# scottjones03/NoisyQuantumSimulator

Measured on AMD Instinct MI355X. Metric: Lindblad param-points/sec (2-atom Rydberg CZ sweep); achieved HBM GB/s vs peak, higher is better.
Workload: dtype f64; 1 GPU; C2: 10k-point (Omega, Delta) LP-square CZ sweep per GPU, medium apparatus, full reference noise model (8 Lindblad channels); points_per_gpu=10000, global_points=10000, parallelism=range-shard x1, method=chebyshev (auto: 16-lane DPP-row propagator kernel, phase frame)

## Files before the change

### noisyquantumsimulator_amd/csrc/ryd_engine.hip

```cpp
#include <hip/hip_runtime.h>

#include <dlfcn.h>

#include <math.h>
#include <stdint.h>
#include <stdio.h>
#include <string.h>

#include <algorithm>
#include <atomic>
#include <chrono>
#include <complex>
#include <condition_variable>
#include <mutex>
#include <string>
#include <thread>
#include <utility>
#include <vector>

#include "../../include/ryd_engine.h"

struct ryd_slot_work {
  void* dbuf = nullptr;
  size_t dcap = 0;
// ... 100 lines not shown
    g.om_re = pulse ? a * q.xr : a;
    g.om_im = pulse ? a * q.xi : 0.0;
    g.dl = q.Dl;
    g.dt = q.tau / (double)n_steps;
  } else if (PROTO == RYD_PROTO_SMOOTH_JP) {
    const double dt = q.tau / (double)n_steps;
    const double tm = (double)s * dt + dt / 2;
    const double ph = q.A * cos(q.wmod * tm - q.phoff);
    double sn, cs;
    sincos(ph, &sn, &cs);
    g.om_re = q.Om * cs;
    g.om_im = q.Om * sn;
    g.dl = q.Dl;
    g.dt = dt;
  } else {
    if (s >= q.nseg) {
      g.om_re = g.om_im = g.dl = g.dt = 0.0;
      return g;
    }
    const double b0 = s == 0 ? 0.0 : col(q.prm, RYD_P_SWT0 + s - 1, q.ld, q.i) / q.Om;
    const double b1 = (s + 1 == q.nseg) ? q.otau / q.Om : col(q.prm, RYD_P_SWT0 + s, q.ld, q.i) / q.Om;
    const double ph = col(q.prm, RYD_P_PHI0 + s, q.ld, q.i);
    double sn, cs;
    sincos(ph, &sn, &cs);
    g.om_re = q.Om * cs;
    g.om_im = q.Om * sn;
    g.dl = 0.0;
    double dt = b1 - b0;
    g.dt = dt < 1e-18 ? 0.0 : dt;
  }
  return g;
}

__device__ __forceinline__ void h_bounds(const Seg& g, double V, double d1, double& emin, double& emax) {
  const double e[3] = {0.0, d1, -g.dl};
  const double w = 0.5 * sqrt(g.om_re * g.om_re + g.om_im * g.om_im);
  emin = 1e300;
  emax = -1e300;
#pragma unroll
  for (int a1 = 0; a1 < 3; ++a1)
#pragma unroll
    for (int a2 = a1; a2 < 3; ++a2) {
      const double E = e[a1] + e[a2] + ((a1 == 2 && a2 == 2) ? V : 0.0);
      const double r = w * ((a1 ? 1.0 : 0.0) + (a2 ? 1.0 : 0.0));
      emin = fmin(emin, E - r);
      emax = fmax(emax, E + r);
    }
}

__device__ __forceinline__ int cheb_terms(double x) {
  if (x < 24.0) {
    double t = 1.0;
    int k = 0;
    do {
      ++k;
      t *= 0.5 * x / (double)k;
    } while (!(t < 1e-18 && (double)k > x));
    return k;
  }
  return (int)ceil(x + 12.0 * cbrt(x) + 10.0);
}

__device__ __forceinline__ int wave_max(int v) {
  v = max(v, __builtin_amdgcn_update_dpp(v, v, 0xB1, 0xF, 0xF, false));
  v = max(v, __builtin_amdgcn_update_dpp(v, v, 0x4E, 0xF, 0xF, false));
  v = max(v, __builtin_amdgcn_update_dpp(v, v, 0x141, 0xF, 0xF, false));
  v = max(v, __builtin_amdgcn_update_dpp(v, v, 0x140, 0xF, 0xF, false));
  const int a = __builtin_amdgcn_readlane(v, 0), b = __builtin_amdgcn_readlane(v, 16);
  const int c = __builtin_amdgcn_readlane(v, 32), d = __builtin_amdgcn_readlane(v, 48);
  return max(max(a, b), max(c, d));
}

struct Gen {
  double g0, g1, mg01, hx, hy, hx2, hy2, hz2, G;
};

__device__ __forceinline__ Gen make_gen(const Seg& g, double d1, const double* r, double s) {
  Gen a;
  const double hx = 0.5 * g.om_re, hy = -0.5 * g.om_im, hz = 0.5 * (d1 + g.dl);
  a.g0 = s * r[1];
// ... 1818 lines not shown
thread_local std::string g_err;

int fail(int code, const std::string& msg) {
  g_err = msg;
  return code;
}

#define HIPCHK(expr)                                                                       \
  do {                                                                                     \
    hipError_t _e = (expr);                                                                \
    if (_e != hipSuccess)                                                                  \
      return fail(RYD_ERR_HIP, std::string(#expr) + ": " + hipGetErrorString(_e));          \
  } while (0)

using KernelFn = void (*)(const double*, int64_t, int64_t, double*, int64_t, double*, int64_t,
                          uint32_t*, int, int);

bool use_propagator(const ryd_batch_desc* d) {
  const bool auto_prop = d->protocol == RYD_PROTO_LP_SQUARE || d->protocol == RYD_PROTO_BANGBANG ||
                         d->protocol == RYD_PROTO_SMOOTH_JP;
  return d->dim == 3 && d->evolution == RYD_EVOL_LINDBLAD &&
         (d->method == RYD_METHOD_CHEB_SQUARING || (d->method == RYD_METHOD_CHEBYSHEV && auto_prop));
}

bool use_sym16(const ryd_batch_desc* d) {
  const char* e = getenv("RYD_SYM16");
  if (e && e[0] == '0') return false;
  return d->dim == 3 && d->evolution == RYD_EVOL_LINDBLAD && d->method == RYD_METHOD_CHEBYSHEV &&
         (d->flags & RYD_FLAG_SYMMETRIC_ATOMS) != 0 &&
         (d->protocol == RYD_PROTO_LP_SQUARE || d->protocol == RYD_PROTO_BANGBANG ||
          d->protocol == RYD_PROTO_SMOOTH_JP);
}

bool use_shaped16(const ryd_batch_desc* d) {
  const char* e = getenv("RYD_SHAPED16");
  if (e && e[0] == '0') return false;
  return d->dim == 3 && d->evolution == RYD_EVOL_LINDBLAD && d->method == RYD_METHOD_CHEBYSHEV &&
         (d->flags & RYD_FLAG_SYMMETRIC_ATOMS) != 0 && d->protocol == RYD_PROTO_LP_SHAPED;
}

bool use_dim4_prop(const ryd_batch_desc* d) {
  const char* e = getenv("RYD_DIM4_PROP");
  if (e && e[0] == '0') return false;
  return d->dim == 4 && d->evolution == RYD_EVOL_LINDBLAD && d->method == RYD_METHOD_CHEBYSHEV &&
         (d->flags & RYD_FLAG_SYMMETRIC_ATOMS) != 0 &&
         (d->protocol == RYD_PROTO_LP_SQUARE || d->protocol == RYD_PROTO_BANGBANG ||
          d->protocol == RYD_PROTO_SMOOTH_JP);
}

bool use_ket_block(const ryd_batch_desc* d) {
  const char* e = getenv("RYD_KET_BLOCK");
  if (e && e[0] == '0') return false;
  return d->evolution == RYD_EVOL_KET && d->method == RYD_METHOD_CHEBYSHEV;
}

KernelFn pick_kernel(const ryd_batch_desc* d) {
  const bool sym = (d->flags & RYD_FLAG_SYMMETRIC_ATOMS) != 0;
  if (d->dim == 4) {
    if (d->evolution == RYD_EVOL_LINDBLAD) {
      switch (d->protocol) {
        case RYD_PROTO_LP_SQUARE:
          return sym ? lindblad4_cheb_kernel<RYD_PROTO_LP_SQUARE, true> : lindblad4_cheb_kernel<RYD_PROTO_LP_SQUARE, false>;
        case RYD_PROTO_LP_SHAPED:
          return sym ? lindblad4_cheb_kernel<RYD_PROTO_LP_SHAPED, true> : lindblad4_cheb_kernel<RYD_PROTO_LP_SHAPED, false>;
        case RYD_PROTO_BANGBANG:
          return sym ? lindblad4_cheb_kernel<RYD_PROTO_BANGBANG, true> : lindblad4_cheb_kernel<RYD_PROTO_BANGBANG, false>;
// ... 155 lines not shown
    int64_t ms = d->max_steps;
    void* args[] = {(void*)&dp, (void*)&n, (void*)&ldp, (void*)&ds, (void*)&lds, (void*)&dm,
                    (void*)&ldm, (void*)&dstat, (void*)&ns, (void*)&sh, (void*)&rt, (void*)&at,
                    (void*)&ms};
    HIPCHK(hipLaunchKernel((const void*)f, dim3((unsigned)blocks), dim3(DP_BLOCK), args, 0, stream));
    return RYD_OK;
  }
  if (use_dim4_prop(d)) {
    using PFn = void (*)(const double*, int64_t, int64_t, double*, int64_t, double*, int64_t, uint32_t*,
                         int, int);
    PFn f = d->protocol == RYD_PROTO_LP_SQUARE ? lindblad4_prop_kernel<RYD_PROTO_LP_SQUARE>
            : d->protocol == RYD_PROTO_SMOOTH_JP ? lindblad4_prop_kernel<RYD_PROTO_SMOOTH_JP>
                                                  : lindblad4_prop_kernel<RYD_PROTO_BANGBANG>;
    const int64_t blocks = (n + D4_PPB - 1) / D4_PPB;
    if (blocks > 0x7fffffffLL) return fail(RYD_ERR_INVALID, "batch too large for one launch");
    int ns = d->n_steps, sh = d->shape;
    void* args[] = {(void*)&dp, (void*)&n, (void*)&ldp, (void*)&ds, (void*)&lds, (void*)&dm,
                    (void*)&ldm, (void*)&dstat, (void*)&ns, (void*)&sh};
    HIPCHK(hipLaunchKernel((const void*)f, dim3((unsigned)blocks), dim3(D4_BLOCK), args, 0, stream));
    return RYD_OK;
  }
  if (use_shaped16(d)) {
    const int64_t blocks = (n + SH_PPW - 1) / SH_PPW;
    if (blocks > 0x7fffffffLL) return fail(RYD_ERR_INVALID, "batch too large for one launch");
    int ns = d->n_steps, sh = d->shape;
    void* args[] = {(void*)&dp, (void*)&n, (void*)&ldp, (void*)&ds, (void*)&lds, (void*)&dm,
                    (void*)&ldm, (void*)&dstat, (void*)&ns, (void*)&sh};
    HIPCHK(hipLaunchKernel((const void*)lindblad_shaped16_kernel<RYD_PROTO_LP_SHAPED>, dim3((unsigned)blocks),
                           dim3(SH_BLOCK), args, 0, stream));
    return RYD_OK;
  }
  if (use_sym16(d)) {
    using SFn = void (*)(const double*, int64_t, int64_t, double*, int64_t, double*, int64_t, uint32_t*,
                         int, int);
    SFn f = d->protocol == RYD_PROTO_LP_SQUARE ? lindblad_sym16_kernel<RYD_PROTO_LP_SQUARE>
            : d->protocol == RYD_PROTO_SMOOTH_JP ? lindblad_sym16_kernel<RYD_PROTO_SMOOTH_JP>
                                                  : lindblad_sym16_kernel<RYD_PROTO_BANGBANG>;
    const int64_t blocks = (n + S16_PPW - 1) / S16_PPW;
    if (blocks > 0x7fffffffLL) return fail(RYD_ERR_INVALID, "batch too large for one launch");
    int ns = d->n_steps, sh = d->shape;
    void* args[] = {(void*)&dp, (void*)&n, (void*)&ldp, (void*)&ds, (void*)&lds, (void*)&dm,
                    (void*)&ldm, (void*)&dstat, (void*)&ns, (void*)&sh};
    HIPCHK(hipLaunchKernel((const void*)f, dim3((unsigned)blocks), dim3(S16_BLOCK), args, 0, stream));
    return RYD_OK;
  }
  if (use_propagator(d) && d->protocol == RYD_PROTO_SMOOTH_JP && jp_split_enabled())
    return launch_jp_split(d, dp, n, ldp, ds, lds, dm, ldm, dstat, stream);
  KernelFn k = pick_kernel(d);
  if (!k) return fail(RYD_ERR_UNSUPPORTED, "no kernel for this descriptor");
  const int64_t blocks = use_propagator(d) ? (n + PPB - 1) / PPB
                        : use_ket_block(d) ? (n + BLOCK - 1) / BLOCK : (4 * n + BLOCK - 1) / BLOCK;
  if (blocks > 0x7fffffffLL) return fail(RYD_ERR_INVALID, "batch too large for one launch");
  int ns = d->n_steps, sh = d->shape;
  void* args[] = {(void*)&dp, (void*)&n, (void*)&ldp, (void*)&ds, (void*)&lds, (void*)&dm,
                  (void*)&ldm, (void*)&dstat, (void*)&ns, (void*)&sh};
  HIPCHK(hipLaunchKernel((const void*)k, dim3((unsigned)blocks), dim3(BLOCK), args, 0, stream));
  return RYD_OK;
}

bool coh_prop_enabled() {
  const char* e = getenv("RYD_COH_PROP");
  return !(e && e[0] == '0');
}

template <int PROTO>
int launch_coherences_proto(const double* dp, int64_t n, int64_t ldp, double* dc, int64_t ldc,
                            uint32_t* dstat, int ns, int sh, hipStream_t stream) {
  if (PROTO != RYD_PROTO_LP_SHAPED && coh_prop_enabled()) {
    const int64_t blocks = (n + CP_NR - 1) / CP_NR;
    if (blocks > 0x7fffffffLL) return fail(RYD_ERR_INVALID, "batch too large for one launch");
    void* args[] = {(void*)&dp, (void*)&n, (void*)&ldp, (void*)&dc, (void*)&ldc, (void*)&dstat, (void*)&ns, (void*)&sh};
    HIPCHK(hipLaunchKernel((const void*)coherence_prop_kernel<PROTO>, dim3((unsigned)blocks), dim3(CP_BLOCK), args, 0,
                           stream));
    return RYD_OK;
  }
// ... 751 lines not shown
```

### noisyquantumsimulator_amd/csrc/ryd_sym16.inc

```

constexpr int S16_BLOCK = 64;
constexpr int S16_PPW = 4;

#ifndef RYD_S16_SETPRIO
#define RYD_S16_SETPRIO 1
#endif
__device__ __forceinline__ bool s16_one_round() {
  return RYD_S16_SETPRIO && gridDim.x <= 256u * 4u * (unsigned)RYD_S16_WAVES;
}
#define S16_PRIO(n) do { if (s16_one_round()) __builtin_amdgcn_s_setprio(n); } while (0)
#ifndef RYD_S16_PRIO_SPLIT
#define RYD_S16_PRIO_SPLIT 1
#endif
#ifdef RYD_S16_PROF
#define S16_MARK(k) (s16_ts[k] = (double)__builtin_readcyclecounter())
#define S16_PROF_ARG , double* s16_ts
#define S16_PROF_PASS , s16_ts
#else
#define S16_MARK(k) ((void)0)
#define S16_PROF_ARG
#define S16_PROF_PASS
#endif

#ifndef RYD_XCD_MAP
#define RYD_XCD_MAP 2
#endif
__device__ __forceinline__ int64_t xcd_block(int64_t b, int64_t nb) {
  if (RYD_XCD_MAP == 0) return b;
  if (RYD_XCD_MAP == 1) {
    const int64_t q = nb / 8, rem = nb % 8, x = b % 8, k = b / 8;
    return x * q + (x < rem ? x : rem) + k;
  }
  const int64_t full = (nb / 32) * 32;
  if (b >= full) return b;
  const int64_t x = b % 8, k = b / 8;
  return ((k / 4) * 8 + x) * 4 + (k % 4);
}

template <int K>
__device__ __forceinline__ double row_bcast(double v) {
  const long long x = __builtin_bit_cast(long long, v);
  const long long y = __builtin_amdgcn_update_dpp(0LL, x, 0x150 + K, 0xF, 0xF, false);
  return __builtin_bit_cast(double, y);
}

template <typename F, int... I>
__device__ __forceinline__ void static_for_impl(F&& f, std::integer_sequence<int, I...>) {
  (f(std::integral_constant<int, I>{}), ...);
}
template <int N, typename F>
__device__ __forceinline__ void static_for(F&& f) {
  static_for_impl(f, std::make_integer_sequence<int, N>{});
}

template <int M, bool NOP>
__device__ __forceinline__ void fmac5_bcast(double& a0, double& a1, double& a2, double& a3, double& a4,
                                            double c0, double c1, double c2, double c3, double c4,
                                            double w) {
  if constexpr (NOP) asm volatile("s_nop 1" ::: "memory");
  asm volatile(
      "v_fmac_f64_dpp %0, %5, %10 row_newbcast:%11 row_mask:0xf bank_mask:0xf\n\t"
      "v_fmac_f64_dpp %1, %6, %10 row_newbcast:%11 row_mask:0xf bank_mask:0xf\n\t"
      "v_fmac_f64_dpp %2, %7, %10 row_newbcast:%11 row_mask:0xf bank_mask:0xf\n\t"
      "v_fmac_f64_dpp %3, %8, %10 row_newbcast:%11 row_mask:0xf bank_mask:0xf\n\t"
      "v_fmac_f64_dpp %4, %9, %10 row_newbcast:%11 row_mask:0xf bank_mask:0xf"
      : "+v"(a0), "+v"(a1), "+v"(a2), "+v"(a3), "+v"(a4)
      : "v"(c0), "v"(c1), "v"(c2), "v"(c3), "v"(c4), "v"(w), "i"(M));
}

// ... 188 lines not shown
  });
}

__device__ __forceinline__ double mrow_re(const Gen& a, int r, double u1, double u2, double u3, double u4,
                                          double o) {
  switch (r) {
    case 0: return fma(a.g0, u2, o);
    case 1: return fma(a.g1, u2, fma(-a.hx2, u4, o));
    case 2: return fma(a.mg01, u2, fma(a.hx2, u4, o));
    case 3: return fma(-a.G, u3, fma(a.hz2, u4, o));
    default: return fma(a.hx, u1 - u2, fma(-a.hz2, u3, fma(-a.G, u4, o)));
  }
}

__device__ __forceinline__ void apply_Lsym_re(const Gen& a, double vs, const double (&t)[15], double (&o)[15]) {
#pragma unroll
  for (int i = 0; i < 5; ++i)
#pragma unroll
    for (int j = i; j < 5; ++j) {
      const int s = sym_index(i, j);
      double acc = mrow_re(a, i, t[tri(1, j)], t[tri(2, j)], t[tri(3, j)], t[tri(4, j)], o[s]);
      o[s] = mrow_re(a, j, t[tri(i, 1)], t[tri(i, 2)], t[tri(i, 3)], t[tri(i, 4)], acc);
    }
  const double v2 = 2.0 * vs;
  const double r23 = t[tri(2, 3)], r24 = t[tri(2, 4)], r33 = t[tri(3, 3)], r34 = t[tri(3, 4)],
               r44 = t[tri(4, 4)];
  o[tri(2, 3)] = fma(-v2, r24, o[tri(2, 3)]);
  o[tri(2, 4)] = fma(v2, r23, o[tri(2, 4)]);
  o[tri(3, 3)] = fma(-v2, r34, o[tri(3, 3)]);
  o[tri(3, 4)] = fma(-vs, r44, fma(vs, r33, o[tri(3, 4)]));
  o[tri(4, 4)] = fma(v2, r34, o[tri(4, 4)]);
}

__device__ __forceinline__ int cheb_terms_small(double x) {
  static_assert(X_BASE_SYM <= 1.0, "cheb_terms_small covers x <= 1 (17 terms)");
  constexpr double TH[17] = {1e-17, 4.4721359549995795e-09, 3.914867641168864e-06, 0.00012446659545769568,
                             0.0010371372893366482, 0.004394290351366487, 0.0125993232817844,
                             0.02822864716464555, 0.05356271212458357, 0.09036001686117834,
                             0.1398168813097236, 0.20262580209060138, 0.2790704614462359,
                             0.36912378048400807, 0.47253426642798413, 0.5888961629494429,
                             0.7177037357024775};
  const double h = 0.5 * x;
  int k = 1;
#pragma unroll
  for (int j = 0; j < 17; ++j) k += (h >= TH[j]) ? 1 : 0;
  return k;
}

constexpr int S16_KS = 20;

template <typename Apply>
__device__ __forceinline__ void cheb_unit16(double (&out)[NS], int r, double x, bool active, Apply apply2Y,
                                            int& nuse, int& nexec) {
  const int kt = active ? cheb_terms_small(x) : -1;
  const int kmax = wave_max(kt);
  if (kmax < 0) {
    asm volatile("" : "+v"(r));
#pragma unroll
    for (int e = 0; e < NS; ++e) out[e] = (e == r) ? 1.0 : 0.0;
    return;
  }
  const int kcut = (kmax + 1) & ~1;
  double bA[NS], bB[NS];
#pragma unroll
  for (int e = 0; e < NS; ++e) bA[e] = bB[e] = 0.0;
  double sel[4];
  {
    const int q = (int)__builtin_amdgcn_mbcnt_hi(~0u, __builtin_amdgcn_mbcnt_lo(~0u, 0u)) & 3;
#pragma unroll
    for (int j = 0; j < 4; ++j) sel[j] = (q == j) ? 1.0 : 0.0;
  }
  auto unit_add = [&](double (&b)[NS], double a) {
    if constexpr (RYD_MASKED_ADD == 3) add_unit15_dpp(b, a, sel);
    else add_unit15<0>(b, a);
  };
  const double i2x = active ? 2.0 / x : 0.0;
  double Jp2 = 0.0, Jp1 = active ? MILLER_SEED : 0.0;
  double S = 2.0 * Jp1;
  {
    const double J = fma(i2x * (double)S16_KS, Jp1, -Jp2);
    Jp2 = Jp1;
    Jp1 = J;
  }
  for (int k = S16_KS - 2; k > kcut; k -= 2) {
    const double Jk = fma(i2x * (double)(k + 1), Jp1, -Jp2);
    Jp2 = Jp1;
    Jp1 = Jk;
    S = fma(2.0, Jk, S);
    const double Jk1 = fma(i2x * (double)k, Jp1, -Jp2);
    Jp2 = Jp1;
    Jp1 = Jk1;
  }
  {
    const int k = kcut;
    const double Jk = fma(i2x * (double)(k + 1), Jp1, -Jp2);
    Jp2 = Jp1;
    Jp1 = Jk;
    S = fma(2.0, Jk, S);
    unit_add(bB, k <= kt ? 2.0 * Jk : 0.0);
    const double Jk1 = fma(i2x * (double)k, Jp1, -Jp2);
    Jp2 = Jp1;
    Jp1 = Jk1;
    unit_add(bA, k - 1 <= kt ? 2.0 * Jk1 : 0.0);
    apply2Y(bB, bA);
  }
  for (int k = kcut - 2; k >= 2; k -= 2) {
    double Jk = fma(i2x * (double)(k + 1), Jp1, -Jp2);
    Jp2 = Jp1;
    Jp1 = Jk;
    S = fma(2.0, Jk, S);
    const double ck = k <= kt ? 2.0 * Jk : 0.0;
    unit_add(bB, ck);
    apply2Y(bA, bB);
    double Jk1 = fma(i2x * (double)k, Jp1, -Jp2);
    Jp2 = Jp1;
    Jp1 = Jk1;
    const double ck1 = k - 1 <= kt ? 2.0 * Jk1 : 0.0;
    unit_add(bA, ck1);
    apply2Y(bB, bA);
  }
  double J0 = fma(i2x, Jp1, -Jp2);
  S += J0;
  if (!active) {
    J0 = 1.0;
    S = 1.0;
  }
  unit_add(bB, J0);
#pragma unroll
  for (int e = 0; e < NS; ++e) bA[e] *= 0.5;
  apply2Y(bA, bB);
  const double inv = 1.0 / S;
#pragma unroll
  for (int e = 0; e < NS; ++e) out[e] = bB[e] * inv;
  if (active) nuse += kt + 1;
  nexec += kcut + 1;
}

__device__ __forceinline__ void segment_phase16(const PointP& q, int s, int n_steps, double& c, double& sn) {
  const double dt = q.tau / (double)n_steps;
  const double tm = (double)s * dt + dt / 2;
  double st, ct;
  fast_sincos(q.wmod * tm - q.phoff, st, ct);
  fast_sincos(q.A * ct, sn, c);
}

constexpr int SEG_M = 10, SEG_Q = 11, SEG_P = 14;
__host__ __device__ constexpr int seg_old(int n) {
  return n == 0 ? 0 : n == 1 ? 1 : n == 2 ? 3 : n == 3 ? 4 : n == 4 ? 2 : n == 5 ? 5 : n == 6 ? 7
       : n == 7 ? 8 : n == 8 ? 10 : n == 9 ? 11 : n == 12 ? 6 : n == 13 ? 9 : 0;
}

__device__ __forceinline__ void build16(double (&u)[NS], double (&Ut)[S16_PPW][NS][16], const PointP& q,
                                        bool valid, bool count, double a, double dl, double dt, int p, int r,
                                        int keep, int& rep, int& nuse, int& nexec, int& nsq,
                                        bool& over_cap, lds_zero_t* zl S16_PROF_ARG) {
  const bool lane_ok = r < NS;
  Seg g;
  g.om_re = a;
  g.om_im = 0.0;
  g.dl = dl;
  g.dt = dt;
  double rsum = 0.0;
#pragma unroll
  for (int k = 0; k < 4; ++k) rsum += fabs(q.gA[k]) + fabs(q.gB[k]);
  double emin, emax;
  h_bounds(g, q.V, q.d1, emin, emax);
  const double omega = (emax - emin) + rsum;
  const double x = omega * dt;
  const bool capped = valid && !(x <= 1e12);
  const bool act = valid && !capped && x > X_SKIP;
  over_cap = over_cap || (count && capped);
  int sqf = 0;
  if (act && x > X_BASE_SYM) {
    int e;
    const double m = frexp(x / X_BASE_SYM, &e);
    sqf = m == 0.5 ? e - 1 : e;
  }
  const double y = act ? ldexp(x, -sqf) : 0.0;
#ifndef RYD_S16_SQ_CAP
  const int sq = sqf > keep ? sqf - keep : 0;
#else
  const int sq = min(sqf > keep ? sqf - keep : 0, RYD_S16_SQ_CAP);
  rep = sqf > keep ? keep : sqf;
#endif
#ifndef RYD_S16_SQ_CAP
  rep = sqf - sq;
#endif
  const double sc = act ? 2.0 / omega : 0.0;
  Gen A = make_gen(g, q.d1, q.gA, sc);
  double vs = sc * 0.5 * q.V;
  if (!act) {
    A = Gen{};
    vs = 0.0;
  }
  double v[NS];
  const int nuse0 = nuse;
  cheb_unit16(v, r, y, act && lane_ok,
              [&](const double (&b)[NS], double (&o)[NS]) { apply_Lsym_re(A, vs, b, o); }, nuse, nexec);
  if (!count) nuse = nuse0;
  S16_MARK(2);
  S16_PRIO(2);
  const int smx = wave_max(sq);
  {
    double w[NS];
    for (int it = 0; it < smx; it += 2) {
      if (RYD_S16_PRIO_SPLIT && it == ((smx >> 1) & ~1)) S16_PRIO(1);
      if (it < sq) square_cols16(v, w, zl);
      if (it + 1 < sq) {
        square_cols16(w, v, zl);
      } else if (it < sq) {
#pragma unroll
        for (int k = 0; k < NS; ++k) v[k] = w[k];
      }
    }
  }
  if (count) nsq += sqf;
  S16_MARK(3);
  S16_PRIO(1);
  wave_sync();
  if (lane_ok) {
    static_for<NS>([&](auto N) {
      constexpr int nn = decltype(N)::value;
      double w;
      if constexpr (nn == SEG_M) w = v[sym_index(3, 3)] - v[sym_index(4, 4)];
      else if constexpr (nn == SEG_Q) w = 2.0 * v[sym_index(3, 4)];
      else if constexpr (nn == SEG_P) w = v[sym_index(3, 3)] + v[sym_index(4, 4)];
      else w = v[seg_old(nn)];
      Ut[p][nn][r] = w;
    });
  }
  wave_sync();
  lds_zero_t* const src = lane_ok ? (lds_zero_t*)&Ut[p][r][0] : zl;
  double R[NS];
#pragma unroll
  for (int m = 0; m < NS; ++m) R[m] = src[m];
  static_for<NS>([&](auto N) {
    constexpr int nn = decltype(N)::value;
    if constexpr (nn == SEG_M) u[nn] = 0.5 * (R[sym_index(3, 3)] - R[sym_index(4, 4)]);
// ... 61 lines not shown
  k.o[0] = r < 5 ? u[0] : 0.0;
#pragma unroll
  for (int m = 1; m < 5; ++m) k.o[m] = h * u[m];
  k.u00 = row_bcast<0>(u[0]);
  return k;
}

#ifndef RYD_JP_WTAB
#define RYD_JP_WTAB 1
#endif
typedef double d2v __attribute__((ext_vector_type(2)));
#ifndef RYD_SEG_LDS_ZERO
#define RYD_SEG_LDS_ZERO 1
#endif
template <bool S00 = true>
__device__ __forceinline__ void seg_apply(const double (&u)[NS], const SegRow01& k, double& t, double& z,
                                          double& s00, lds_zero_t* zl = nullptr) {
  double acc = 0.0, acc1 = 0.0;
  if constexpr (RYD_SEG_LDS_ZERO != 0 && !S00) {
    asm volatile("" ::: "memory");
    acc = zl[0];
    asm volatile("" ::: "memory");
    acc1 = zl[1];
  }
  dot5_bcast<0>(acc, t, u[0], u[1], u[2], u[3], u[4]);
  dot5_bcast<5, false>(acc, t, u[5], u[6], u[7], u[8], u[9]);
  dot5_bcast<10, false>(acc, t, u[10], u[11], u[12], u[13], u[14]);
  dot5_bcast<0>(acc1, z, k.o[0], k.o[1], k.o[2], k.o[3], k.o[4]);
  t = acc;
  if constexpr (S00) s00 = k.u00 * s00;
  z = acc1;
}

__device__ __forceinline__ void sym16_epilogue(double t, double z, double s00, double cp, double sp, bool valid,
                                               bool over_cap, int nuse, int nexec, int nsq, int l, int p,
                                               int64_t blk, int64_t n, double* __restrict__ st, int64_t lds,
                                               double* __restrict__ sm, int64_t ldm,
                                               uint32_t* __restrict__ status, double (&Ut)[S16_PPW][NS][16]
                                               S16_PROF_ARG);

typedef __attribute__((address_space(1))) char s16_gchar;
typedef __attribute__((address_space(1))) double s16_gdouble;
template <int PROTO>
__device__ __forceinline__ PointP load_point16(const double* __restrict__ prm, int64_t ldp, int64_t i0,
                                               unsigned po8) {
  unsigned off = po8;
  if constexpr (PROTO != RYD_PROTO_SMOOTH_JP)
    asm("" : "+v"(off));
  PointP q = load_point_with<PROTO>([&](int f) {
    const char* base = reinterpret_cast<const char*>(prm + ((int64_t)f * ldp + i0));
    asm("" : "+s"(base));
    const s16_gchar* gbase = (const s16_gchar*)base;
    return *reinterpret_cast<const s16_gdouble*>(gbase + off);
  });
  q.prm = prm;
  q.ld = ldp;
  q.i = i0 + (int64_t)(po8 >> 3);
  return q;
}

template <int PROTO>
__global__ __launch_bounds__(S16_BLOCK) __attribute__((amdgpu_waves_per_eu(PROTO == RYD_PROTO_BANGBANG ? 3 : RYD_S16_WAVES, 8))) void
lindblad_sym16_kernel(const double* __restrict__ prm, int64_t n, int64_t ldp, double* __restrict__ st,
                      int64_t lds, double* __restrict__ sm, int64_t ldm, uint32_t* __restrict__ status,
                      int n_steps, int shape) {
  __shared__ __attribute__((aligned(16))) double Ut[S16_PPW][NS][16];
  static_assert(sizeof(Ut) >= sizeof(double) * S16_PPW * 4 * NC, "output staging must fit in Ut");
  (void)shape;
#ifdef RYD_S16_PROF
  double s16_ts[10];
  s16_ts[8] = (double)__builtin_amdgcn_s_memrealtime();
  S16_MARK(0);
#endif
  __shared__ double Zl[16];
  const int l = threadIdx.x;
  const int p = l >> 4, r = l & 15;
  if (l < 16) Zl[l] = 0.0;
  const int64_t b0 = xcd_block(blockIdx.x, gridDim.x) * S16_PPW;
  const int64_t i0 = b0 < n ? b0 : n - 1;
  const int64_t last = n - 1 - i0;
  const unsigned po8 = 8u * (unsigned)min(p, last < S16_PPW - 1 ? (int)last : S16_PPW - 1);
  const PointP q0 = load_point16<PROTO>(prm, ldp, i0, po8);
  const bool valid = point_valid<PROTO>(q0, n_steps);
  const bool frame_ok =
      !(PROTO == RYD_PROTO_LP_SQUARE) || !valid || fabs(q0.xr * q0.xr + q0.xi * q0.xi - 1.0) <= 1e-14;
  S16_MARK(1);
  S16_PRIO(3);
#ifndef RYD_S16_TAIL_PRIO
#define RYD_S16_TAIL_PRIO 3
#endif
  if (RYD_S16_TAIL_PRIO && !s16_one_round() &&
      blockIdx.x + 256u * 4u * (unsigned)RYD_S16_WAVES >= gridDim.x)
    __builtin_amdgcn_s_setprio(RYD_S16_TAIL_PRIO);
  double t = (r == sym_index(1, 1)) ? 1.0 : 0.0;
  double z = (r == 1) ? 1.0 : 0.0;
  double s00 = 1.0;
  double u[NS];
  double cp = 1.0, sp = 0.0;
  int nuse = 0, nexec = 0, nsq = 0;
  bool over_cap = false;
  const int nseg = n_segments<PROTO>(n_steps);

  if constexpr (PROTO == RYD_PROTO_SMOOTH_JP) {
    double ph_c, ph_s, dt;
    double th_c, th_s, dc, ds;
    {
      const PointP& q = q0;
      dt = q.tau / (double)n_steps;
      int rep0;
      build16(u, Ut, q, valid, valid, q.Om, q.Dl, dt, p, r, 0, rep0, nuse, nexec, nsq, over_cap,
              (lds_zero_t*)Zl S16_PROF_PASS);
      fast_sincos(q.wmod * ((double)r * dt + dt / 2) - q.phoff, th_s, th_c);
      fast_sincos(16.0 * (q.wmod * dt), ds, dc);
    }
    const SegRow01 k1 = seg_row01(u, r);
    const SegRot rw = seg_rot(r);
    d2v* wtab = reinterpret_cast<d2v*>(&Ut[0][0][0]);
    static_assert(sizeof(Ut) >= sizeof(d2v) * S16_PPW * 16 * 5, "weight table must fit in Ut");
    const bool th = r == 2 || r == 3 || r == 6 || r == 7 || r == 8 || r == 9;
    const int wtyp = th ? 1 + (r & 1) : (r == SEG_M || r == SEG_Q) ? 3 + (r & 1) : 0;
    if constexpr (RYD_JP_WTAB != 0) {
      wave_sync();
      wtab[(p * 16 + r) * 5] = d2v{1.0, 0.0};
    }
    for (int s0 = 0; s0 < nseg; s0 += 16) {
      {
        const double* pp = prm;
        asm volatile("" : "+s"(pp));
        const PointP q = load_point16<PROTO>(pp, ldp, i0, po8);
        double cth = th_c;
        if (s0 + 16 > nseg) {
          double st, ct;
          fast_sincos(q.wmod * ((double)(nseg - 1) * dt + dt / 2) - q.phoff, st, ct);
          if (s0 + r >= nseg) cth = ct;
        }
        fast_sincos(q.A * cth, ph_s, ph_c);
        const double tc = fma(th_c, dc, -th_s * ds);
        th_s = fma(th_s, dc, th_c * ds);
        th_c = tc;
      }
      double pc = row_shr1(ph_c), ps = row_shr1(ph_s);
      if (r == 0) {
        pc = cp;
// ... 15 lines not shown
        constexpr int j = decltype(J)::value;
        if (s0 + j < nseg) {
          double al, be;
          if constexpr (RYD_JP_WTAB != 0) {
            const d2v w = wtab[(p * 16 + j) * 5 + wtyp];
            al = w.x;
            be = w.y;
          } else {
            al = rw.wI;
            be = 0.0;
            fmac2_bcast<j>(al, C2, rw.w2, cr, rw.wT);
            fmac2_bcast<j>(be, S2, rw.b2, sr, rw.bT);
          }
          t = fma(al, t, be * quad_swap(t));
          z = fma(al, z, be * quad_swap(z));
          seg_apply<false>(u, k1, t, z, s00, (lds_zero_t*)Zl);
        }
      });
    }
    {
      double b = k1.u00, acc = 1.0;
      for (int e = nseg; e > 0; e >>= 1) {
        if (e & 1) acc *= b;
        b *= b;
      }
      s00 = acc;
    }
  } else {
    __shared__ double Sv[S16_PPW][16][2];
    __shared__ double Sp[S16_PPW][8];
    __shared__ int Sc[S16_PPW][2];
    constexpr int KEEP = PROTO == RYD_PROTO_LP_SQUARE ? RYD_LP_UNSQUARED : 0;
    int rep = 0, nrep = 0;
    if (nseg > 0) {
      const PointP& q = q0;
      double a, c, sn, dl, dt;
      bool hold;
      seg_polar<PROTO>(q, 0, n_steps, frame_ok, a, c, sn, dl, dt, hold);
      build16(u, Ut, q, valid, valid, a, dl, dt, p, r, KEEP, rep, nuse, nexec, nsq, over_cap,
              (lds_zero_t*)Zl S16_PROF_PASS);
      nrep = wave_max(rep);
      if (r == 0) {
        Sp[p][5] = a;
        Sp[p][6] = dt;
      }
      const SegRow01 k1 = seg_row01(u, r);
      t = u[sym_index(1, 1)];
      z = k1.o[1];
      s00 = k1.u00;
      for (int j = 1; j < (1 << nrep); ++j) {
        if (j < (1 << rep)) seg_apply(u, k1, t, z, s00);
      }
      if (!hold) {
        cp = c;
        sp = sn;
      }
      wave_sync();
    }
    for (int s = 1; s < nseg; ++s) {
      const double* pp = prm;
      asm volatile("" : "+s"(pp));
      const PointP q = load_point16<PROTO>(pp, ldp, i0, po8);
      double a, c, sn, dl, dt;
      bool hold;
      seg_polar<PROTO>(q, s, n_steps, frame_ok, a, c, sn, dl, dt, hold);
      const bool need = valid && !(a == Sp[p][5] && dt == Sp[p][6]);
      if (__builtin_amdgcn_ballot_w64(need) != 0) {
        Sv[p][r][0] = t;
        Sv[p][r][1] = z;
        if (r == 0) {
          Sp[p][0] = s00;
          Sp[p][1] = cp;
          Sp[p][2] = sp;
          Sc[p][0] = nuse;
          Sc[p][1] = nsq;
        }
        int nu = 0, nq = 0;
        const double* pb = pp;
        if constexpr (PROTO == RYD_PROTO_LP_SQUARE) asm volatile("" : "+s"(pb));
        const PointP qb = load_point16<PROTO>(pb, ldp, i0, po8);
        build16(u, Ut, qb, valid, need, a, dl, dt, p, r, KEEP, rep, nu, nexec, nq, over_cap,
                (lds_zero_t*)Zl S16_PROF_PASS);
        nrep = wave_max(rep);
        t = Sv[p][r][0];
        z = Sv[p][r][1];
        s00 = Sp[p][0];
        cp = Sp[p][1];
        sp = Sp[p][2];
        nuse = Sc[p][0] + nu;
        nsq = Sc[p][1] + nq;
        wave_sync();
        if (r == 0) {
          Sp[p][5] = a;
          Sp[p][6] = dt;
        }
        wave_sync();
        const double* pq = prm;
        asm volatile("" : "+s"(pq));
        seg_polar<PROTO>(load_point16<PROTO>(pq, ldp, i0, po8), s, n_steps, frame_ok, a, c, sn, dl, dt, hold);
      }
      if (hold) {
        c = cp;
        sn = sp;
      }
      const double cr = cp * c + sp * sn, sr = sp * c - cp * sn;
      const SegRow01 k1 = seg_row01(u, r);
      rotate_state(t, z, cr, sr, seg_rot(r));
      seg_apply(u, k1, t, z, s00);
      for (int j = 1; j < (1 << nrep); ++j) {
        if (j < (1 << rep)) seg_apply(u, k1, t, z, s00);
      }
      cp = c;
      sp = sn;
    }
  }
  S16_MARK(5);
  {
    const int lid = (int)__builtin_amdgcn_mbcnt_hi(~0u, __builtin_amdgcn_mbcnt_lo(~0u, 0u));
    int pl = lid >> 4;
    asm volatile("" : "+v"(pl));
    const int64_t b2 = xcd_block(blockIdx.x, gridDim.x);
    return sym16_epilogue(t, z, s00, cp, sp, valid, over_cap, nuse, nexec, nsq, lid, pl, b2, n, st, lds, sm, ldm,
                          status, Ut S16_PROF_PASS);
  }
}

__device__ __forceinline__ void sym16_epilogue(double t, double z, double s00, double cp, double sp, bool valid,
                                               bool over_cap, int nuse, int nexec, int nsq, int l, int p,
                                               int64_t blk, int64_t n, double* __restrict__ st, int64_t lds,
                                               double* __restrict__ sm, int64_t ldm,
                                               uint32_t* __restrict__ status, double (&Ut)[S16_PPW][NS][16]
                                               S16_PROF_ARG) {
  const int r = l & 15;
  const bool lane_ok = r < NS;
  const int64_t ip = blk * S16_PPW + p;
  const int64_t i = ip < n ? ip : n - 1;
  rotate_state(t, z, cp, sp, seg_rot(r));
  {
    const double mv = row_bcast<SEG_M>(t), pv = row_bcast<SEG_P>(t);
    if (r == SEG_M) t = 0.5 * (pv + mv);
    if (r == SEG_Q) t = 0.5 * t;
    if (r == SEG_P) t = 0.5 * (pv - mv);
  }
  double (*Ro)[4][NC] = reinterpret_cast<double (*)[4][NC]>(&Ut[0][0][0]);
  wave_sync();
#pragma unroll
  for (int e = r; e < 4 * NC; e += 16) (&Ro[p][0][0])[e] = 0.0;
  wave_sync();
  if (lane_ok) {
    const int ia = (int)((0x0421332211100000ull >> (4 * r)) & 15);
    const int ja = (int)((0x0422434343124310ull >> (4 * r)) & 15);
    Ro[p][3][5 * ia + ja] = t;
    Ro[p][3][5 * ja + ia] = t;
  }
  if (r < 5) {
    const int mz = (int)((0x24310u >> (4 * r)) & 15);
    Ro[p][1][mz] = z;
    Ro[p][2][5 * mz] = z;
  }
  if (r == 0) Ro[p][0][0] = s00;
  wave_sync();
  const int64_t i0 = blk * S16_PPW;
  {
    const int cc = l & 15, pp = cc >> 2, k = cc & 3;
    double* dst = st + 4 * i0 + cc;
    const bool in = i0 + pp < n;
    double v[7];
#pragma unroll
    for (int j = 0; j < 7; ++j) {
      const int row = (l >> 4) + 4 * j;
      v[j] = row < NC ? Ro[pp][k][row] : 0.0;
    }
#pragma unroll
    for (int j = 0; j < 7; ++j) {
      const int row = (l >> 4) + 4 * j;
      if (in && row < NC) dst[(int64_t)row * lds] = v[j];
    }
  }
#ifdef RYD_S16_PROF
  S16_MARK(7);
#endif
  static_assert(RYD_S_POP0 == 0 && RYD_S_AVG_POP == 12 && RYD_S_AVG_F == 15 && RYD_S_NMV_USEFUL == 16 &&
                    RYD_S_NMV_EXEC == 17 && RYD_S_TRACE11 == 18 && RYD_S_NSQUARE == 19,
                "summary columns are written by lane index");
  const bool ok = (!lane_ok || isfinite(t)) && (r >= 5 || isfinite(z)) && isfinite(s00);
  const uint64_t bad = __builtin_amdgcn_ballot_w64(!ok);
  const bool fin = ((bad >> (16 * p)) & 0xFFFFull) == 0;
  const double z1 = row_bcast<1>(z), t11 = row_bcast<5>(t);
  const double t00 = row_bcast<0>(t), t01 = row_bcast<1>(t);
  const double t02 = row_bcast<4>(t), t12 = row_bcast<12>(t);
  const double t22 = row_bcast<13>(t);
  const double tr11 = ((((((((0.0 + t00) + t01) + t02) + t01) + t11) + t12) + t02) + t12) + t22;
  if (ip < n) {
    const double nan = __builtin_nan("");
    const double avg = 0.25 * (s00 + z1 + z1 + t11);
    double v = nan;
    if (r < 4) v = r == 0 ? s00 : (r == 3 ? t11 : z1);
    else if (r == RYD_S_AVG_POP || r == RYD_S_AVG_F) v = avg;
#ifdef RYD_S16_PROF
    S16_MARK(6);
    s16_ts[9] = (double)__builtin_amdgcn_s_memrealtime();
    if (r >= 4 && r < 10) v = s16_ts[r - 3] - s16_ts[0];
    if (r == 10 || r == 11) v = s16_ts[r - 2];
    if (r == 13) v = (double)__builtin_amdgcn_s_getreg((4) | (0 << 6) | (31 << 11));
    if (r == 14) v = s16_ts[7] - s16_ts[0];
#endif
    sm[(int64_t)r * ldm + i] = v;
    if (r < 4) {
      const double c = r == 0 ? (double)(NS * nuse) : r == 1 ? (double)(16 * nexec) : r == 2 ? tr11 : (double)nsq;
      sm[(int64_t)(RYD_S_NMV_USEFUL + r) * ldm + i] = c;
    }
    if (r == 0) {
      uint32_t stat = valid ? 0u : RYD_STATUS_BAD_INPUT;
      if (over_cap) stat |= RYD_STATUS_STEP_CAP;
      if (!fin) stat |= RYD_STATUS_NONFINITE;
      status[i] = stat;
    }
  }
}
```

Baseline: 404.4 million points/s.

## Trim sym16 kernel overheads: 32-bit store offsets, LP-square fast path, DPP reductions

Bundles several micro-optimisations in the sym16 Lindblad kernel. Epilogue stores now use scalar base pointers plus 32-bit lane offsets when the strides fit, which saves 64-bit address arithmetic. For LP-square, later segments skip reloading point parameters and recomputing the segment, and the spectral-bound sqrt is skipped when the amplitude is in a plain range. Smaller changes: a 16-lane DPP max that finishes with readlane, zero-initialising accumulators from LDS, bit-cast conversion of the Chebyshev order to double, and a bounded Chebyshev term count. Each adds code paths and edge-case conditions that need correctness checks.

```diff
diff --git a/noisyquantumsimulator_amd/csrc/ryd_engine.hip b/noisyquantumsimulator_amd/csrc/ryd_engine.hip
--- a/noisyquantumsimulator_amd/csrc/ryd_engine.hip
+++ b/noisyquantumsimulator_amd/csrc/ryd_engine.hip
@@ -156,9 +156,9 @@
   return g;
 }
 
-__device__ __forceinline__ void h_bounds(const Seg& g, double V, double d1, double& emin, double& emax) {
-  const double e[3] = {0.0, d1, -g.dl};
-  const double w = 0.5 * sqrt(g.om_re * g.om_re + g.om_im * g.om_im);
+__device__ __forceinline__ void h_bounds_w(double w, double dl, double V, double d1, double& emin,
+                                           double& emax) {
+  const double e[3] = {0.0, d1, -dl};
   emin = 1e300;
   emax = -1e300;
 #pragma unroll
@@ -170,6 +170,10 @@
       emin = fmin(emin, E - r);
       emax = fmax(emax, E + r);
     }
+}
+
+__device__ __forceinline__ void h_bounds(const Seg& g, double V, double d1, double& emin, double& emax) {
+  h_bounds_w(0.5 * sqrt(g.om_re * g.om_re + g.om_im * g.om_im), g.dl, V, d1, emin, emax);
 }
 
 __device__ __forceinline__ int cheb_terms(double x) {
@@ -2054,6 +2058,11 @@
           d->protocol == RYD_PROTO_SMOOTH_JP);
 }
 
+bool sym16_store32_enabled() {
+  const char* e = getenv("RYD_S16_STORE64");
+  return !(e && e[0] == '1');
+}
+
 bool use_shaped16(const ryd_batch_desc* d) {
   const char* e = getenv("RYD_SHAPED16");
   if (e && e[0] == '0') return false;
@@ -2275,15 +2284,17 @@
   }
   if (use_sym16(d)) {
     using SFn = void (*)(const double*, int64_t, int64_t, double*, int64_t, double*, int64_t, uint32_t*,
-                         int, int);
+                         int, int, int);
     SFn f = d->protocol == RYD_PROTO_LP_SQUARE ? lindblad_sym16_kernel<RYD_PROTO_LP_SQUARE>
             : d->protocol == RYD_PROTO_SMOOTH_JP ? lindblad_sym16_kernel<RYD_PROTO_SMOOTH_JP>
                                                   : lindblad_sym16_kernel<RYD_PROTO_BANGBANG>;
     const int64_t blocks = (n + S16_PPW - 1) / S16_PPW;
     if (blocks > 0x7fffffffLL) return fail(RYD_ERR_INVALID, "batch too large for one launch");
     int ns = d->n_steps, sh = d->shape;
+    int st32 = sym16_store32_enabled() && lds >= 0 && ldm >= 0 && lds <= (0x1fffffffLL - 15) / 3 &&
+               ldm <= (0x1fffffffLL - 3) / 15;
     void* args[] = {(void*)&dp, (void*)&n, (void*)&ldp, (void*)&ds, (void*)&lds, (void*)&dm,
-                    (void*)&ldm, (void*)&dstat, (void*)&ns, (void*)&sh};
+                    (void*)&ldm, (void*)&dstat, (void*)&ns, (void*)&sh, (void*)&st32};
     HIPCHK(hipLaunchKernel((const void*)f, dim3((unsigned)blocks), dim3(S16_BLOCK), args, 0, stream));
     return RYD_OK;
   }
diff --git a/noisyquantumsimulator_amd/csrc/ryd_sym16.inc b/noisyquantumsimulator_amd/csrc/ryd_sym16.inc
--- a/noisyquantumsimulator_amd/csrc/ryd_sym16.inc
+++ b/noisyquantumsimulator_amd/csrc/ryd_sym16.inc
@@ -35,6 +35,16 @@
   if (b >= full) return b;
   const int64_t x = b % 8, k = b / 8;
   return ((k / 4) * 8 + x) * 4 + (k % 4);
+}
+
+__device__ __forceinline__ int wave_max16(int v) {
+  v = max(v, __builtin_amdgcn_mov_dpp(v, 0xB1, 0xF, 0xF, true));
+  v = max(v, __builtin_amdgcn_mov_dpp(v, 0x4E, 0xF, 0xF, true));
+  v = max(v, __builtin_amdgcn_mov_dpp(v, 0x141, 0xF, 0xF, true));
+  v = max(v, __builtin_amdgcn_mov_dpp(v, 0x140, 0xF, 0xF, true));
+  const int a = __builtin_amdgcn_readlane(v, 0), b = __builtin_amdgcn_readlane(v, 16);
+  const int c = __builtin_amdgcn_readlane(v, 32), d = __builtin_amdgcn_readlane(v, 48);
+  return max(max(a, b), max(c, d));
 }
 
 template <int K>
@@ -289,6 +299,7 @@
   o[tri(4, 4)] = fma(v2, r34, o[tri(4, 4)]);
 }
 
+template <bool BOUNDED = false>
 __device__ __forceinline__ int cheb_terms_small(double x) {
   static_assert(X_BASE_SYM <= 1.0, "cheb_terms_small covers x <= 1 (17 terms)");
   constexpr double TH[17] = {1e-17, 4.4721359549995795e-09, 3.914867641168864e-06, 0.00012446659545769568,
@@ -297,20 +308,28 @@
                              0.1398168813097236, 0.20262580209060138, 0.2790704614462359,
                              0.36912378048400807, 0.47253426642798413, 0.5888961629494429,
                              0.7177037357024775};
+  constexpr double HMAX = BOUNDED ? 0.5 * X_BASE_SYM * (1.0 + 1e-12) : 1.0;
   const double h = 0.5 * x;
   int k = 1;
 #pragma unroll
-  for (int j = 0; j < 17; ++j) k += (h >= TH[j]) ? 1 : 0;
+  for (int j = 0; j < 17; ++j)
+    if (TH[j] <= HMAX) k += (h >= TH[j]) ? 1 : 0;
   return k;
 }
 
 constexpr int S16_KS = 20;
+
+__device__ __forceinline__ double order_f64(int k) {
+  const int e = 31 - __builtin_clz((unsigned)k);
+  const unsigned hi = ((unsigned)(1023 + e) << 20) | (((unsigned)k << (20 - e)) & 0xFFFFFu);
+  return __builtin_bit_cast(double, (unsigned long long)hi << 32);
+}
 
 template <typename Apply>
 __device__ __forceinline__ void cheb_unit16(double (&out)[NS], int r, double x, bool active, Apply apply2Y,
-                                            int& nuse, int& nexec) {
-  const int kt = active ? cheb_terms_small(x) : -1;
-  const int kmax = wave_max(kt);
+                                            int& nuse, int& nexec, lds_zero_t* zl) {
+  const int kt = active ? cheb_terms_small<true>(x) : -1;
+  const int kmax = wave_max16(kt);
   if (kmax < 0) {
     asm volatile("" : "+v"(r));
 #pragma unroll
@@ -319,8 +338,17 @@
   }
   const int kcut = (kmax + 1) & ~1;
   double bA[NS], bB[NS];
-#pragma unroll
-  for (int e = 0; e < NS; ++e) bA[e] = bB[e] = 0.0;
+  asm volatile("" ::: "memory");
+#pragma unroll
+  for (int e = 0; e < NS; ++e) {
+    bA[e] = zl[e];
+    asm volatile("" ::: "memory");
+  }
+#pragma unroll
+  for (int e = 0; e < NS; ++e) {
+    bB[e] = zl[e];
+    asm volatile("" ::: "memory");
+  }
   double sel[4];
   {
     const int q = (int)__builtin_amdgcn_mbcnt_hi(~0u, __builtin_amdgcn_mbcnt_lo(~0u, 0u)) & 3;
@@ -340,36 +368,36 @@
     Jp1 = J;
   }
   for (int k = S16_KS - 2; k > kcut; k -= 2) {
-    const double Jk = fma(i2x * (double)(k + 1), Jp1, -Jp2);
+    const double Jk = fma(i2x * order_f64(k + 1), Jp1, -Jp2);
     Jp2 = Jp1;
     Jp1 = Jk;
     S = fma(2.0, Jk, S);
-    const double Jk1 = fma(i2x * (double)k, Jp1, -Jp2);
+    const double Jk1 = fma(i2x * order_f64(k), Jp1, -Jp2);
     Jp2 = Jp1;
     Jp1 = Jk1;
   }
   {
     const int k = kcut;
-    const double Jk = fma(i2x * (double)(k + 1), Jp1, -Jp2);
+    const double Jk = fma(i2x * order_f64(k + 1), Jp1, -Jp2);
     Jp2 = Jp1;
     Jp1 = Jk;
     S = fma(2.0, Jk, S);
     unit_add(bB, k <= kt ? 2.0 * Jk : 0.0);
-    const double Jk1 = fma(i2x * (double)k, Jp1, -Jp2);
+    const double Jk1 = fma(i2x * order_f64(k), Jp1, -Jp2);
     Jp2 = Jp1;
     Jp1 = Jk1;
     unit_add(bA, k - 1 <= kt ? 2.0 * Jk1 : 0.0);
     apply2Y(bB, bA);
   }
   for (int k = kcut - 2; k >= 2; k -= 2) {
-    double Jk = fma(i2x * (double)(k + 1), Jp1, -Jp2);
+    double Jk = fma(i2x * order_f64(k + 1), Jp1, -Jp2);
     Jp2 = Jp1;
     Jp1 = Jk;
     S = fma(2.0, Jk, S);
     const double ck = k <= kt ? 2.0 * Jk : 0.0;
     unit_add(bB, ck);
     apply2Y(bA, bB);
-    double Jk1 = fma(i2x * (double)k, Jp1, -Jp2);
+    double Jk1 = fma(i2x * order_f64(k), Jp1, -Jp2);
     Jp2 = Jp1;
     Jp1 = Jk1;
     const double ck1 = k - 1 <= kt ? 2.0 * Jk1 : 0.0;
@@ -409,7 +437,7 @@
 
 __device__ __forceinline__ void build16(double (&u)[NS], double (&Ut)[S16_PPW][NS][16], const PointP& q,
                                         bool valid, bool count, double a, double dl, double dt, int p, int r,
-                                        int keep, int& rep, int& nuse, int& nexec, int& nsq,
+                                        int keep, int& rep, int& nrep, int& nuse, int& nexec, int& nsq,
                                         bool& over_cap, lds_zero_t* zl S16_PROF_ARG) {
   const bool lane_ok = r < NS;
   Seg g;
@@ -420,8 +448,16 @@
   double rsum = 0.0;
 #pragma unroll
   for (int k = 0; k < 4; ++k) rsum += fabs(q.gA[k]) + fabs(q.gB[k]);
+  const double fa = fabs(a);
+  const bool plain = (fa >= 0x1p-500 && fa <= 0x1p500) || fa == 0.0;
+  double hw = 0.5 * fa;
+  if (__builtin_amdgcn_ballot_w64(!plain) != 0) {
+    double ar = g.om_re;
+    asm volatile("" : "+v"(ar));
+    hw = 0.5 * sqrt(ar * ar + g.om_im * g.om_im);
+  }
   double emin, emax;
-  h_bounds(g, q.V, q.d1, emin, emax);
+  h_bounds_w(hw, g.dl, q.V, q.d1, emin, emax);
   const double omega = (emax - emin) + rsum;
   const double x = omega * dt;
   const bool capped = valid && !(x <= 1e12);
@@ -453,14 +489,20 @@
   double v[NS];
   const int nuse0 = nuse;
   cheb_unit16(v, r, y, act && lane_ok,
-              [&](const double (&b)[NS], double (&o)[NS]) { apply_Lsym_re(A, vs, b, o); }, nuse, nexec);
+              [&](const double (&b)[NS], double (&o)[NS]) { apply_Lsym_re(A, vs, b, o); }, nuse, nexec, zl);
   if (!count) nuse = nuse0;
   S16_MARK(2);
   S16_PRIO(2);
-  const int smx = wave_max(sq);
+  const int sfm = wave_max16(sqf);
+  nrep = sfm > keep ? keep : sfm;
+#ifndef RYD_S16_SQ_CAP
+  const int smx = sfm > keep ? sfm - keep : 0;
+#else
+  const int smx = min(sfm > keep ? sfm - keep : 0, RYD_S16_SQ_CAP);
+#endif
   {
-    double w[NS];
     for (int it = 0; it < smx; it += 2) {
+      double w[NS];
       if (RYD_S16_PRIO_SPLIT && it == ((smx >> 1) & ~1)) S16_PRIO(1);
       if (it < sq) square_cols16(v, w, zl);
       if (it + 1 < sq) {
@@ -588,12 +630,12 @@
   z = acc1;
 }
 
-__device__ __forceinline__ void sym16_epilogue(double t, double z, double s00, double cp, double sp, bool valid,
-                                               bool over_cap, int nuse, int nexec, int nsq, int l, int p,
-                                               int64_t blk, int64_t n, double* __restrict__ st, int64_t lds,
-                                               double* __restrict__ sm, int64_t ldm,
-                                               uint32_t* __restrict__ status, double (&Ut)[S16_PPW][NS][16]
-                                               S16_PROF_ARG);
+__device__ __forceinline__ void sym16_epilogue(double t, double z, double s00, double cp, double sp,
+                                               const SegRot& rw, bool valid, bool over_cap, int nuse, int nexec,
+                                               int nsq, int l, int p, int64_t blk, int64_t n,
+                                               double* __restrict__ st, int64_t lds, double* __restrict__ sm,
+                                               int64_t ldm, uint32_t* __restrict__ status, bool st32,
+                                               double (&Ut)[S16_PPW][NS][16] S16_PROF_ARG);
 
 typedef __attribute__((address_space(1))) char s16_gchar;
 typedef __attribute__((address_space(1))) double s16_gdouble;
@@ -619,7 +661,7 @@
 __global__ __launch_bounds__(S16_BLOCK) __attribute__((amdgpu_waves_per_eu(PROTO == RYD_PROTO_BANGBANG ? 3 : RYD_S16_WAVES, 8))) void
 lindblad_sym16_kernel(const double* __restrict__ prm, int64_t n, int64_t ldp, double* __restrict__ st,
                       int64_t lds, double* __restrict__ sm, int64_t ldm, uint32_t* __restrict__ status,
-                      int n_steps, int shape) {
+                      int n_steps, int shape, int st32) {
   __shared__ __attribute__((aligned(16))) double Ut[S16_PPW][NS][16];
   static_assert(sizeof(Ut) >= sizeof(double) * S16_PPW * 4 * NC, "output staging must fit in Ut");
   (void)shape;
@@ -656,6 +698,7 @@
   int nuse = 0, nexec = 0, nsq = 0;
   bool over_cap = false;
   const int nseg = n_segments<PROTO>(n_steps);
+  SegRot rw_out = {};
 
   if constexpr (PROTO == RYD_PROTO_SMOOTH_JP) {
     double ph_c, ph_s, dt;
@@ -664,7 +707,8 @@
       const PointP& q = q0;
       dt = q.tau / (double)n_steps;
       int rep0;
-      build16(u, Ut, q, valid, valid, q.Om, q.Dl, dt, p, r, 0, rep0, nuse, nexec, nsq, over_cap,
+      int nrep0;
+      build16(u, Ut, q, valid, valid, q.Om, q.Dl, dt, p, r, 0, rep0, nrep0, nuse, nexec, nsq, over_cap,
               (lds_zero_t*)Zl S16_PROF_PASS);
       fast_sincos(q.wmod * ((double)r * dt + dt / 2) - q.phoff, th_s, th_c);
       fast_sincos(16.0 * (q.wmod * dt), ds, dc);
@@ -746,19 +790,21 @@
     __shared__ int Sc[S16_PPW][2];
     constexpr int KEEP = PROTO == RYD_PROTO_LP_SQUARE ? RYD_LP_UNSQUARED : 0;
     int rep = 0, nrep = 0;
+    SegRow01 k1 = {};
     if (nseg > 0) {
       const PointP& q = q0;
       double a, c, sn, dl, dt;
       bool hold;
       seg_polar<PROTO>(q, 0, n_steps, frame_ok, a, c, sn, dl, dt, hold);
-      build16(u, Ut, q, valid, valid, a, dl, dt, p, r, KEEP, rep, nuse, nexec, nsq, over_cap,
+      build16(u, Ut, q, valid, valid, a, dl, dt, p, r, KEEP, rep, nrep, nuse, nexec, nsq, over_cap,
               (lds_zero_t*)Zl S16_PROF_PASS);
-      nrep = wave_max(rep);
-      if (r == 0) {
-        Sp[p][5] = a;
-        Sp[p][6] = dt;
-      }
-      const SegRow01 k1 = seg_row01(u, r);
+      if constexpr (PROTO != RYD_PROTO_LP_SQUARE) {
+        if (r == 0) {
+          Sp[p][5] = a;
+          Sp[p][6] = dt;
+        }
+      }
+      k1 = seg_row01(u, r);
       t = u[sym_index(1, 1)];
       z = k1.o[1];
       s00 = k1.u00;
@@ -772,54 +818,65 @@
       wave_sync();
     }
     for (int s = 1; s < nseg; ++s) {
-      const double* pp = prm;
-      asm volatile("" : "+s"(pp));
-      const PointP q = load_point16<PROTO>(pp, ldp, i0, po8);
       double a, c, sn, dl, dt;
-      bool hold;
-      seg_polar<PROTO>(q, s, n_steps, frame_ok, a, c, sn, dl, dt, hold);
-      const bool need = valid && !(a == Sp[p][5] && dt == Sp[p][6]);
-      if (__builtin_amdgcn_ballot_w64(need) != 0) {
-        Sv[p][r][0] = t;
-        Sv[p][r][1] = z;
-        if (r == 0) {
-          Sp[p][0] = s00;
-          Sp[p][1] = cp;
-          Sp[p][2] = sp;
-          Sc[p][0] = nuse;
-          Sc[p][1] = nsq;
+      bool hold = false;
+      bool general = true;
+      if constexpr (PROTO == RYD_PROTO_LP_SQUARE) {
+        general = __builtin_amdgcn_ballot_w64(!frame_ok) != 0;
+        c = q0.xr;
+        sn = q0.xi;
+      }
+      if (general) {
+        const double* pp = prm;
+        asm volatile("" : "+s"(pp));
+        const PointP q = load_point16<PROTO>(pp, ldp, i0, po8);
+        seg_polar<PROTO>(q, s, n_steps, frame_ok, a, c, sn, dl, dt, hold);
+        const bool need = PROTO == RYD_PROTO_LP_SQUARE ? valid && !(a == q.Om && dt == q.tau)
+                                                       : valid && !(a == Sp[p][5] && dt == Sp[p][6]);
+        if (__builtin_amdgcn_ballot_w64(need) != 0) {
+          Sv[p][r][0] = t;
+          Sv[p][r][1] = z;
+          if (r == 0) {
+            Sp[p][0] = s00;
+            Sp[p][1] = cp;
+            Sp[p][2] = sp;
+            Sc[p][0] = nuse;
+            Sc[p][1] = nsq;
+          }
+          int nu = 0, nq = 0;
+          const double* pb = pp;
+          if constexpr (PROTO == RYD_PROTO_LP_SQUARE) asm volatile("" : "+s"(pb));
+          const PointP qb = load_point16<PROTO>(pb, ldp, i0, po8);
+          build16(u, Ut, qb, valid, need, a, dl, dt, p, r, KEEP, rep, nrep, nu, nexec, nq, over_cap,
+                  (lds_zero_t*)Zl S16_PROF_PASS);
+          t = Sv[p][r][0];
+          z = Sv[p][r][1];
+          s00 = Sp[p][0];
+          cp = Sp[p][1];
+          sp = Sp[p][2];
+          nuse = Sc[p][0] + nu;
+          nsq = Sc[p][1] + nq;
+          wave_sync();
+          if constexpr (PROTO != RYD_PROTO_LP_SQUARE) {
+            if (r == 0) {
+              Sp[p][5] = a;
+              Sp[p][6] = dt;
+            }
+            wave_sync();
+          }
+          const double* pq = prm;
+          asm volatile("" : "+s"(pq));
+          seg_polar<PROTO>(load_point16<PROTO>(pq, ldp, i0, po8), s, n_steps, frame_ok, a, c, sn, dl, dt, hold);
+          k1 = seg_row01(u, r);
         }
-        int nu = 0, nq = 0;
-        const double* pb = pp;
-        if constexpr (PROTO == RYD_PROTO_LP_SQUARE) asm volatile("" : "+s"(pb));
-        const PointP qb = load_point16<PROTO>(pb, ldp, i0, po8);
-        build16(u, Ut, qb, valid, need, a, dl, dt, p, r, KEEP, rep, nu, nexec, nq, over_cap,
-                (lds_zero_t*)Zl S16_PROF_PASS);
-        nrep = wave_max(rep);
-        t = Sv[p][r][0];
-        z = Sv[p][r][1];
-        s00 = Sp[p][0];
-        cp = Sp[p][1];
-        sp = Sp[p][2];
-        nuse = Sc[p][0] + nu;
-        nsq = Sc[p][1] + nq;
-        wave_sync();
-        if (r == 0) {
-          Sp[p][5] = a;
-          Sp[p][6] = dt;
-        }
-        wave_sync();
-        const double* pq = prm;
-        asm volatile("" : "+s"(pq));
-        seg_polar<PROTO>(load_point16<PROTO>(pq, ldp, i0, po8), s, n_steps, frame_ok, a, c, sn, dl, dt, hold);
       }
       if (hold) {
         c = cp;
         sn = sp;
       }
       const double cr = cp * c + sp * sn, sr = sp * c - cp * sn;
-      const SegRow01 k1 = seg_row01(u, r);
-      rotate_state(t, z, cr, sr, seg_rot(r));
+      rw_out = seg_rot(r);
+      rotate_state(t, z, cr, sr, rw_out);
       seg_apply(u, k1, t, z, s00);
       for (int j = 1; j < (1 << nrep); ++j) {
         if (j < (1 << rep)) seg_apply(u, k1, t, z, s00);
@@ -834,22 +891,23 @@
     int pl = lid >> 4;
     asm volatile("" : "+v"(pl));
     const int64_t b2 = xcd_block(blockIdx.x, gridDim.x);
-    return sym16_epilogue(t, z, s00, cp, sp, valid, over_cap, nuse, nexec, nsq, lid, pl, b2, n, st, lds, sm, ldm,
-                          status, Ut S16_PROF_PASS);
-  }
-}
-
-__device__ __forceinline__ void sym16_epilogue(double t, double z, double s00, double cp, double sp, bool valid,
-                                               bool over_cap, int nuse, int nexec, int nsq, int l, int p,
-                                               int64_t blk, int64_t n, double* __restrict__ st, int64_t lds,
-                                               double* __restrict__ sm, int64_t ldm,
-                                               uint32_t* __restrict__ status, double (&Ut)[S16_PPW][NS][16]
-                                               S16_PROF_ARG) {
+    if constexpr (PROTO != RYD_PROTO_LP_SQUARE) rw_out = seg_rot(lid & 15);
+    return sym16_epilogue(t, z, s00, cp, sp, rw_out, valid, over_cap, nuse, nexec, nsq, lid, pl, b2, n, st, lds, sm,
+                          ldm, status, st32 != 0, Ut S16_PROF_PASS);
+  }
+}
+
+__device__ __forceinline__ void sym16_epilogue(double t, double z, double s00, double cp, double sp,
+                                               const SegRot& rw, bool valid, bool over_cap, int nuse, int nexec,
+                                               int nsq, int l, int p, int64_t blk, int64_t n,
+                                               double* __restrict__ st, int64_t lds, double* __restrict__ sm,
+                                               int64_t ldm, uint32_t* __restrict__ status, bool st32,
+                                               double (&Ut)[S16_PPW][NS][16] S16_PROF_ARG) {
   const int r = l & 15;
   const bool lane_ok = r < NS;
   const int64_t ip = blk * S16_PPW + p;
   const int64_t i = ip < n ? ip : n - 1;
-  rotate_state(t, z, cp, sp, seg_rot(r));
+  rotate_state(t, z, cp, sp, rw);
   {
     const double mv = row_bcast<SEG_M>(t), pv = row_bcast<SEG_P>(t);
     if (r == SEG_M) t = 0.5 * (pv + mv);
@@ -877,18 +935,33 @@
   const int64_t i0 = blk * S16_PPW;
   {
     const int cc = l & 15, pp = cc >> 2, k = cc & 3;
-    double* dst = st + 4 * i0 + cc;
     const bool in = i0 + pp < n;
     double v[7];
 #pragma unroll
-    for (int j = 0; j < 7; ++j) {
-      const int row = (l >> 4) + 4 * j;
-      v[j] = row < NC ? Ro[pp][k][row] : 0.0;
-    }
-#pragma unroll
-    for (int j = 0; j < 7; ++j) {
-      const int row = (l >> 4) + 4 * j;
-      if (in && row < NC) dst[(int64_t)row * lds] = v[j];
+    for (int j = 0; j < 7; ++j)
+      v[j] = (&Ro[pp][k][0])[(l >> 4) + 4 * j];
+    static_assert(NC == 25, "rows l/16 + 4 j: j < 6 always inside, j = 6 on the first 16 lanes only");
+    if (st32) {
+      const unsigned lo = 8u * ((unsigned)cc + (unsigned)(l >> 4) * (unsigned)lds);
+      if (in) {
+#pragma unroll
+        for (int j = 0; j < 7; ++j) {
+          if (j < 6 || l < 16) {
+            char* bj = reinterpret_cast<char*>(st + (4 * i0 + 4 * j * lds));
+            asm("" : "+s"(bj));
+            *reinterpret_cast<s16_gdouble*>((s16_gchar*)bj + lo) = v[j];
+          }
+        }
+      }
+    } else {
+      double* dst = st + 4 * i0 + cc;
+      if (in) {
+#pragma unroll
+        for (int j = 0; j < 7; ++j) {
+          const int row = (l >> 4) + 4 * j;
+          if (j < 6 || l < 16) dst[(int64_t)row * lds] = v[j];
+        }
+      }
     }
   }
 #ifdef RYD_S16_PROF
@@ -919,16 +992,27 @@
     if (r == 13) v = (double)__builtin_amdgcn_s_getreg((4) | (0 << 6) | (31 << 11));
     if (r == 14) v = s16_ts[7] - s16_ts[0];
 #endif
-    sm[(int64_t)r * ldm + i] = v;
-    if (r < 4) {
-      const double c = r == 0 ? (double)(NS * nuse) : r == 1 ? (double)(16 * nexec) : r == 2 ? tr11 : (double)nsq;
-      sm[(int64_t)(RYD_S_NMV_USEFUL + r) * ldm + i] = c;
-    }
-    if (r == 0) {
-      uint32_t stat = valid ? 0u : RYD_STATUS_BAD_INPUT;
-      if (over_cap) stat |= RYD_STATUS_STEP_CAP;
-      if (!fin) stat |= RYD_STATUS_NONFINITE;
-      status[i] = stat;
-    }
-  }
-}
+    const int ci = r == 0 ? NS * nuse : r == 1 ? 16 * nexec : nsq;
+    const double c = r == 2 ? tr11 : (double)ci;
+    uint32_t stat = valid ? 0u : RYD_STATUS_BAD_INPUT;
+    if (over_cap) stat |= RYD_STATUS_STEP_CAP;
+    if (!fin) stat |= RYD_STATUS_NONFINITE;
+    if (st32) {
+      char* b0 = reinterpret_cast<char*>(sm + i0);
+      char* b1 = reinterpret_cast<char*>(sm + (RYD_S_NMV_USEFUL * ldm + i0));
+      char* b2 = reinterpret_cast<char*>(status + i0);
+      asm("" : "+s"(b0));
+      asm("" : "+s"(b1));
+      asm("" : "+s"(b2));
+      const unsigned lo = 8u * ((unsigned)r * (unsigned)ldm + (unsigned)p);
+      *reinterpret_cast<s16_gdouble*>((s16_gchar*)b0 + lo) = v;
+      if (r < 4) *reinterpret_cast<s16_gdouble*>((s16_gchar*)b1 + lo) = c;
+      if (r == 0)
+        *reinterpret_cast<__attribute__((address_space(1))) uint32_t*>((s16_gchar*)b2 + 4u * (unsigned)p) = stat;
+    } else {
+      sm[(int64_t)r * ldm + i] = v;
+      if (r < 4) sm[(int64_t)(RYD_S_NMV_USEFUL + r) * ldm + i] = c;
+      if (r == 0) status[i] = stat;
+    }
+  }
+}
```

Result: faster. 418.8 million points/s, median of 6 (+3.6%).
